# ShuhangGu/DASR

Measured on AMD Instinct MI355X. Metric: SR train images/sec (4x, 128->512), higher is better.
Workload: dtype bf16 MFMA operands, fp32 accumulate / fp32 residual stream

## Files before the change

### dasr_amd/csrc/common.h

```cpp
#pragma once
#include <hip/hip_runtime.h>
#include <hip/hip_ext.h>
#include <stdint.h>
#include "../../include/dasr_hip.h"

typedef __bf16 bf16_t;
typedef __attribute__((ext_vector_type(8))) __bf16 bf16x8;
typedef __attribute__((ext_vector_type(4))) __bf16 bf16x4;
typedef __attribute__((ext_vector_type(4))) short s16x4;
typedef _Float16 f16_t;
typedef __attribute__((ext_vector_type(8))) _Float16 f16x8;
typedef __attribute__((ext_vector_type(4))) _Float16 f16x4;
typedef __attribute__((ext_vector_type(16))) float f32x16;
typedef __attribute__((ext_vector_type(4))) float f32x4;
typedef __attribute__((ext_vector_type(4))) unsigned int u32x4;
typedef __attribute__((ext_vector_type(2))) unsigned int u32x2;

#define DASR_LDS __attribute__((address_space(3)))

#define HIP_TRY(expr)                                   \
    do {                                                \
        hipError_t _e = (expr);                         \
        if (_e != hipSuccess) return (int)_e;           \
    } while (0)

__device__ __forceinline__ float bf16_to_f32(bf16_t v) { return (float)v; }

__device__ __forceinline__ bf16_t f32_to_bf16(float v) { return (bf16_t)v; }

__device__ __forceinline__ void split_bf16(float v, bf16_t& hi, bf16_t& lo) {
    hi = (bf16_t)v;
    lo = (bf16_t)(v - (float)hi);
}

__device__ __forceinline__ void split_f16(float v, bf16_t& hi, bf16_t& lo) {
    const f16_t h = (f16_t)v;
    hi = __builtin_bit_cast(bf16_t, h);
    lo = __builtin_bit_cast(bf16_t, (f16_t)(v - (float)h));
}

template <bool F16>
__device__ __forceinline__ f32x16 mfma16(bf16x8 a, bf16x8 b, f32x16 c) {
    if constexpr (F16) return __builtin_amdgcn_mfma_f32_32x32x16_f16(__builtin_bit_cast(f16x8, a), __builtin_bit_cast(f16x8, b), c, 0, 0, 0);
    else return __builtin_amdgcn_mfma_f32_32x32x16_bf16(a, b, c, 0, 0, 0);
}

__device__ __forceinline__ float wave_sum(float v) {
#pragma unroll
    for (int o = 32; o > 0; o >>= 1) v += __shfl_xor(v, o, 64);
    return v;
}

static inline hipStream_t as_stream(void* s) { return (hipStream_t)s; }

struct dasr_red {
    float* part;
    unsigned* ticket;
};
dasr_red dasr_red_scratch(const void* key_acc, hipStream_t s, unsigned nblocks, int k);
int dasr_red_error();

template <int K>
__device__ __forceinline__ void grid_sum_commit(const dasr_red r, const float (&v)[K], float* const (&acc)[K], const float (&coef)[K]) {
    if (!r.part) return;
    __shared__ unsigned gs_last;
    __shared__ float gs_red[K][4];
    const unsigned nb = gridDim.x;
    if (threadIdx.x == 0) {
#pragma unroll
        for (int k = 0; k < K; ++k) __hip_atomic_store(r.part + (size_t)k * nb + blockIdx.x, v[k], __ATOMIC_RELAXED, __HIP_MEMORY_SCOPE_AGENT);
        asm volatile("s_waitcnt vmcnt(0)" ::: "memory");
        gs_last = __hip_atomic_fetch_add(r.ticket, 1u, __ATOMIC_RELAXED, __HIP_MEMORY_SCOPE_AGENT) == nb - 1u;
    }
    __syncthreads();
    if (!gs_last) return;
#pragma unroll
    for (int k = 0; k < K; ++k) {
        float s = 0.f;
        for (unsigned i = threadIdx.x; i < nb; i += 256u) s += __hip_atomic_load(r.part + (size_t)k * nb + i, __ATOMIC_RELAXED, __HIP_MEMORY_SCOPE_AGENT);
        s = wave_sum(s);
        if ((threadIdx.x & 63) == 0) gs_red[k][threadIdx.x >> 6] = s;
    }
    __syncthreads();
    if (threadIdx.x == 0) {
#pragma unroll
        for (int k = 0; k < K; ++k)
            if (acc[k]) atomicAdd(acc[k], ((gs_red[k][0] + gs_red[k][1]) + (gs_red[k][2] + gs_red[k][3])) * coef[k]);
        __hip_atomic_store(r.ticket, 0u, __ATOMIC_RELAXED, __HIP_MEMORY_SCOPE_AGENT);
    }
}

bool dasr_prof_slot(const char* tag, hipEvent_t* e0, hipEvent_t* e1);
#define DASR_LAUNCH_TAG(tag, kfn, grid, block, lds, s, ...)                                         \
    do {                                                                                            \
        hipEvent_t _e0 = nullptr, _e1 = nullptr;                                                    \
        if (dasr_prof_slot(tag, &_e0, &_e1)) hipExtLaunchKernelGGL(kfn, grid, block, lds, s, _e0, _e1, 0, __VA_ARGS__); \
        else hipLaunchKernelGGL(kfn, grid, block, lds, s, __VA_ARGS__);                             \
    } while (0)
#define DASR_LAUNCH(kfn, ...) DASR_LAUNCH_TAG(#kfn, kfn, __VA_ARGS__)
```

### dasr_amd/csrc/misc.hip

```cpp
#include "common.h"
#include <string.h>
#include <atomic>
#include <condition_variable>
#include <map>
#include <mutex>
#include <thread>
#include <tuple>

namespace {

__global__ void pack_kernel(const dasr_pack_desc* __restrict__ descs, int ndesc, long long total,
                            const long long* __restrict__ prefix, const float* __restrict__ params, bf16_t* __restrict__ packed) {
    const long long gid = (long long)blockIdx.x * blockDim.x + threadIdx.x;
    if (gid >= total) return;
    int lo = 0, hi = ndesc - 1;
    while (lo < hi) {
        const int mid = (lo + hi + 1) >> 1;
        if (prefix[mid] <= gid) lo = mid; else hi = mid - 1;
    }
    const dasr_pack_desc& D = descs[lo];
    long long q = gid - prefix[lo];
    const int lane = q & 63;
    q >>= 6;
    const int mi = q % D.mt;
    q /= D.mt;
    const int tap = q % D.ntaps;
    q /= D.ntaps;
    const int nchunks = D.cin_pad >> 4;
    const int ckv = q % nchunks;
    const int mg = q / nchunks;
    const int oc = (mg * D.mt + mi) * 32 + (lane & 31);
    const int kreal = D.fmt >= 3 ? nchunks / 3 : nchunks;
    const int part = ckv / kreal, ck = ckv - part * kreal;
    const int c0 = ck * 16 + 8 * (lane >> 5);
    bf16x8 vh, vl;
#pragma unroll
    for (int e = 0; e < 8; ++e) {
        const int cin = c0 + e;
        float v = 0.f;
        if (oc < D.cout) {
            for (int s = 0; s < D.nseg; ++s) {
                const dasr_pack_seg& S = D.seg[s];
                const int ci = cin - S.cin_start;
                if (ci >= 0 && ci < S.cin_len) {
                    const int st = D.tapmap[tap];
                    const unsigned msk = tap < 16 ? D.tapmask[tap] : 0u;
                    const bool okc = !S.transpose || ci < S.src_cout;
                    const long long base = !S.transpose ? S.src_off + ((long long)oc * S.src_cin + S.src_c0 + ci) * D.src_ntaps
                                                        : S.src_off + ((long long)ci * S.src_cin + S.src_c0 + oc) * D.src_ntaps;
                    if (msk && okc) {
                        float acc = 0.f;
                        for (int k = 0; k < D.src_ntaps && k < 16; ++k)
                            if (msk & (1u << k)) acc += params[base + k];
                        v = acc;
                    } else if (st >= 0 && okc) {
                        v = params[base + st];
                    }
                }
            }
        }
        bf16_t h, l;
        split_bf16(v, h, l);
        if (D.fmt == 1) h = __builtin_bit_cast(bf16_t, (f16_t)v);
        if (D.fmt == 2 || D.fmt == 3) split_f16(v, h, l);
        if (D.fmt >= 3 && part == 2) h = l;
        vh[e] = h;
        vl[e] = l;
    }
    const long long o = D.dst_off + (gid - prefix[lo]) * 8;
    *(bf16x8*)(packed + o) = vh;
    if (D.lo_off) *(bf16x8*)(packed + o + D.lo_off) = vl;
}

__global__ void nchw_to_blocked_kernel(const float* __restrict__ src, int N, int C, int H, int W, dasr_tensor df, dasr_tensor db) {
    const int ncb = (C + 15) >> 4;
    const long long total = (long long)N * ncb * H * W;
    const long long i = (long long)blockIdx.x * blockDim.x + threadIdx.x;
    if (i >= total) return;
    const int x = i % W;
    long long t = i / W;
    const int y = t % H;
    t /= H;
    const int cb = t % ncb;
    const int n = t / ncb;
    float v[16];
#pragma unroll
    for (int j = 0; j < 16; ++j) {
        const int c = cb * 16 + j;
        v[j] = c < C ? src[(((long long)n * C + c) * H + y) * W + x] : 0.f;
    }
    const size_t po = ((size_t)y * W + x) * 16;
    if (df.p) {
        float* d = (float*)df.p + (size_t)n * df.n_stride + (size_t)cb * df.cb_stride + po;
#pragma unroll
        for (int j = 0; j < 4; ++j) ((f32x4*)d)[j] = f32x4{v[4 * j], v[4 * j + 1], v[4 * j + 2], v[4 * j + 3]};
    }
    if (db.p) {
        bf16_t* d = (bf16_t*)db.p + (size_t)n * db.n_stride + (size_t)cb * db.cb_stride + po;
        bf16x8 a, b;
#pragma unroll
        for (int j = 0; j < 8; ++j) {
            a[j] = (bf16_t)v[j];
            b[j] = (bf16_t)v[8 + j];
        }
        ((bf16x8*)d)[0] = a;
        ((bf16x8*)d)[1] = b;
    }
}

__global__ void blocked_to_nchw_kernel(dasr_tensor s, int N, int C, int H, int W, float* __restrict__ dst) {
    const long long total = (long long)N * C * H * W;
    const long long i = (long long)blockIdx.x * blockDim.x + threadIdx.x;
    if (i >= total) return;
    const int x = i % W;
    long long t = i / W;
    const int y = t % H;
    t /= H;
    const int c = t % C;
    const int n = t / C;
    dst[i] = ((const float*)s.p)[(size_t)n * s.n_stride + (size_t)(c >> 4) * s.cb_stride + ((size_t)y * W + x) * 16 + (c & 15)];
}

__global__ void l1_loss_kernel(dasr_tensor sr, const float* __restrict__ hr, const float* __restrict__ wm, int N, int C, int H, int W,
                               float coef, float* loss_acc, dasr_tensor grad, int accumulate, float gscale, dasr_red rs) {
    const long long total = (long long)N * H * W;
    const long long i = (long long)blockIdx.x * blockDim.x + threadIdx.x;
    float part = 0.f;
    if (i < total) {
        const int x = i % W;
        long long t = i / W;
        const int y = t % H;
        const int n = t / H;
        const size_t po = ((size_t)y * W + x) * 16;
        const float* s = (const float*)sr.p + (size_t)n * sr.n_stride + po;
        const float wgt = wm ? wm[((long long)n * H + y) * W + x] : 1.f;
        float g[16];
#pragma unroll
        for (int j = 0; j < 16; ++j) g[j] = 0.f;
        for (int c = 0; c < C; ++c) {
            const float d = s[c] - hr[(((long long)n * C + c) * H + y) * W + x];
            if (accumulate & 2) {
                part += wgt * d * d;
                g[c] = 2.f * coef * wgt * d;
            } else {
                part += wgt * fabsf(d);
                g[c] = coef * wgt * (d > 0.f ? 1.f : (d < 0.f ? -1.f : 0.f));
            }
        }
        if (grad.p && (accumulate & 4)) {
            f16_t* gp = (f16_t*)grad.p + (size_t)n * grad.n_stride + po;
            for (int j = 0; j < (C + 3) / 4; ++j) {
                f16x4 o;
#pragma unroll
                for (int e = 0; e < 4; ++e) o[e] = (f16_t)(g[4 * j + e] * gscale);
                ((f16x4*)gp)[j] = o;
            }
        } else if (grad.p) {
            float* gp = (float*)grad.p + (size_t)n * grad.n_stride + po;
#pragma unroll
            for (int j = 0; j < 4; ++j) {
                f32x4 o = {g[4 * j], g[4 * j + 1], g[4 * j + 2], g[4 * j + 3]};
                if (accumulate & 1) o += ((const f32x4*)gp)[j];
                ((f32x4*)gp)[j] = o;
            }
        }
    }
    part = wave_sum(part);
    __shared__ float red[4];
    if ((threadIdx.x & 63) == 0) red[threadIdx.x >> 6] = part;
    __syncthreads();
    const float v[1] = {red[0] + red[1] + red[2] + red[3]};
    float* const acc[1] = {loss_acc};
    const float cf[1] = {coef};
    grid_sum_commit<1>(rs, v, acc, cf);
}

__global__ void downsum2x_kernel(dasr_tensor src, int N, int C, int H, int W, dasr_tensor mask, int mask_f32, float slope,
                                 dasr_tensor df, dasr_tensor db) {
    const int ncb = (C + 15) >> 4;
    const long long total = (long long)N * ncb * H * W * 4;
    const long long gi = (long long)blockIdx.x * blockDim.x + threadIdx.x;
    if (gi >= total) return;
    const int q = gi & 3;
    const long long i = gi >> 2;
    const int x = i % W;
    long long t = i / W;
    const int y = t % H;
    t /= H;
    const int cb = t % ncb;
    const int n = t / ncb;
    const float* s = (const float*)src.p + (size_t)n * src.n_stride + (size_t)cb * src.cb_stride + q * 4;
    const int W2 = 2 * W;
    f32x4 a = *(const f32x4*)(s + ((size_t)(2 * y) * W2 + 2 * x) * 16);
    a += *(const f32x4*)(s + ((size_t)(2 * y) * W2 + 2 * x + 1) * 16);
    a += *(const f32x4*)(s + ((size_t)(2 * y + 1) * W2 + 2 * x) * 16);
    a += *(const f32x4*)(s + ((size_t)(2 * y + 1) * W2 + 2 * x + 1) * 16);
    const size_t po = ((size_t)y * W + x) * 16 + q * 4;
    if (mask.p) {
        const size_t mo = (size_t)n * mask.n_stride + (size_t)cb * mask.cb_stride + po;
        float m[4];
        if (mask_f32) {
            const f32x4 mv = *(const f32x4*)((const float*)mask.p + mo);
            for (int j = 0; j < 4; ++j) m[j] = mv[j];
        } else {
            const bf16x4 mv = *(const bf16x4*)((const bf16_t*)mask.p + mo);
            for (int j = 0; j < 4; ++j) m[j] = (float)mv[j];
        }
        for (int j = 0; j < 4; ++j) a[j] = m[j] > 0.f ? a[j] : a[j] * slope;
    }
    if (df.p) *(f32x4*)((float*)df.p + (size_t)n * df.n_stride + (size_t)cb * df.cb_stride + po) = a;
    if (db.p) {
        bf16x4 o;
        for (int j = 0; j < 4; ++j) o[j] = (bf16_t)a[j];
        *(bf16x4*)((bf16_t*)db.p + (size_t)n * db.n_stride + (size_t)cb * db.cb_stride + po) = o;
    }
}

__global__ void axpby_kernel(dasr_tensor x, float a, dasr_tensor z, float b, int N, int C, int H, int W, dasr_tensor of,
                             dasr_tensor ob, float gamma, dasr_tensor mask, float slope, const float* slope_ptr) {
    const int ncb = (C + 15) >> 4;
    const long long per_plane = (long long)H * W * 4;
    const long long total = (long long)N * ncb * per_plane;
    const long long gi = (long long)blockIdx.x * blockDim.x + threadIdx.x;
    if (gi >= total) return;
    const long long e = (gi % per_plane) * 4;
    long long t = gi / per_plane;
    const int cb = t % ncb;
    const int n = t / ncb;
    f32x4 v = *(const f32x4*)((const float*)x.p + (size_t)n * x.n_stride + (size_t)cb * x.cb_stride + e) * a;
    if (z.p) v += *(const f32x4*)((const float*)z.p + (size_t)n * z.n_stride + (size_t)cb * z.cb_stride + e) * b;
    if (mask.p) {
        const float sl = slope_ptr ? *slope_ptr : slope;
        const f32x4 mv = *(const f32x4*)((const float*)mask.p + (size_t)n * mask.n_stride + (size_t)cb * mask.cb_stride + e);
        for (int j = 0; j < 4; ++j) v[j] = mv[j] > 0.f ? v[j] : v[j] * sl;
    }
    if (of.p) *(f32x4*)((float*)of.p + (size_t)n * of.n_stride + (size_t)cb * of.cb_stride + e) = v;
    if (ob.p) {
        bf16x4 o;
        for (int j = 0; j < 4; ++j) o[j] = (bf16_t)(v[j] * gamma);
        *(bf16x4*)((bf16_t*)ob.p + (size_t)n * ob.n_stride + (size_t)cb * ob.cb_stride + e) = o;
    }
}

__global__ void adam_kernel(float* __restrict__ p, const float* __restrict__ g, float* __restrict__ m, float* __restrict__ v,
                            long long n, float step_size, float beta1, float beta2, float eps, float wd, float inv_sqrt_bc2, int* __restrict__ nonfinite,
                            const int* __restrict__ gate) {
    if (gate && *gate != 0) return;
    bool bad = false;
    for (long long i = (long long)blockIdx.x * blockDim.x + threadIdx.x; i < n; i += (long long)gridDim.x * blockDim.x) {
        float gi = g[i];
        bad |= !(fabsf(gi) <= 3.0e38f);
        const float pi = p[i];
        if (wd != 0.f) gi += wd * pi;
        const float mi = beta1 * m[i] + (1.f - beta1) * gi;
        const float vi = beta2 * v[i] + (1.f - beta2) * gi * gi;
        m[i] = mi;
        v[i] = vi;
        const float denom = sqrtf(vi) * inv_sqrt_bc2 + eps;
        p[i] = pi - step_size * (mi / denom);
    }
    if (nonfinite && __any(bad) && (threadIdx.x & 63) == 0) atomicOr(nonfinite, 1);
}

__global__ void add_flat_kernel(float* __restrict__ y, const float* __restrict__ x, long long n) {
    for (long long i = (long long)blockIdx.x * blockDim.x + threadIdx.x; i < n; i += (long long)gridDim.x * blockDim.x) y[i] += x[i];
}

__global__ void fill_kernel(float* p, long long n, float v) {
    for (long long i = (long long)blockIdx.x * blockDim.x + threadIdx.x; i < n; i += (long long)gridDim.x * blockDim.x) p[i] = v;
}

inline unsigned blocks_for(long long total, int bs = 256) { return (unsigned)((total + bs - 1) / bs); }

}

extern "C" int dasr_pack_weights(const dasr_pack_desc* descs_dev, int32_t ndesc, int64_t total_pieces, const int64_t* piece_prefix_dev,
                                 const float* params_flat, void* packed, void* stream) {
    if (ndesc <= 0 || total_pieces <= 0) return DASR_EINVAL;
    DASR_LAUNCH(pack_kernel, dim3(blocks_for(total_pieces)), dim3(256), 0, as_stream(stream), descs_dev, ndesc,
                       (long long)total_pieces, (const long long*)piece_prefix_dev, params_flat, (bf16_t*)packed);
    return (int)hipGetLastError();
}

extern "C" int dasr_nchw_to_blocked(const float* src, int32_t N, int32_t C, int32_t H, int32_t W, dasr_tensor dst_f32,
                                    dasr_tensor dst_bf16, void* stream) {
    const long long total = (long long)N * ((C + 15) / 16) * H * W;
    if (total <= 0) return DASR_EINVAL;
    DASR_LAUNCH(nchw_to_blocked_kernel, dim3(blocks_for(total)), dim3(256), 0, as_stream(stream), src, N, C, H, W, dst_f32, dst_bf16);
    return (int)hipGetLastError();
}

extern "C" int dasr_blocked_to_nchw(dasr_tensor src, int32_t N, int32_t C, int32_t H, int32_t W, float* dst, void* stream) {
    const long long total = (long long)N * C * H * W;
    if (total <= 0) return DASR_EINVAL;
    DASR_LAUNCH(blocked_to_nchw_kernel, dim3(blocks_for(total)), dim3(256), 0, as_stream(stream), src, N, C, H, W, dst);
    return (int)hipGetLastError();
}

extern "C" int dasr_l1_loss(dasr_tensor sr, const float* hr_nchw, const float* weight_map, int32_t N, int32_t C, int32_t H, int32_t W,
                            float coef, float* loss_acc, dasr_tensor grad, int32_t accumulate, float grad_scale, void* stream) {
    const long long total = (long long)N * H * W;
    if (total <= 0 || C > 16) return DASR_EINVAL;
    if ((accumulate & 4) && (accumulate & 1)) return DASR_EINVAL;
    const dasr_red rs = dasr_red_scratch(loss_acc, as_stream(stream), blocks_for(total), 1);
    if (loss_acc && !rs.part) return dasr_red_error();
    DASR_LAUNCH(l1_loss_kernel, dim3(blocks_for(total)), dim3(256), 0, as_stream(stream), sr, hr_nchw, weight_map, N, C, H, W, coef,
                       loss_acc, grad, accumulate, grad_scale != 0.f ? grad_scale : 1.f, rs);
    return (int)hipGetLastError();
}

extern "C" int dasr_downsum2x(dasr_tensor src, int32_t N, int32_t C, int32_t H, int32_t W, dasr_tensor mask, int32_t mask_f32,
                              float slope, dasr_tensor dst_f32, dasr_tensor dst_bf16, void* stream) {
    const long long total = (long long)N * ((C + 15) / 16) * H * W * 4;
    if (total <= 0) return DASR_EINVAL;
    DASR_LAUNCH(downsum2x_kernel, dim3(blocks_for(total)), dim3(256), 0, as_stream(stream), src, N, C, H, W, mask, mask_f32, slope,
                       dst_f32, dst_bf16);
    return (int)hipGetLastError();
}

__device__ __forceinline__ float f32_rounded(float v) {
    asm("" : "+v"(v));
    return v;
}

__global__ void cvt_f16_kernel(dasr_tensor x, int N, int C, int H, int W, float scale, dasr_tensor y) {
    const int ncb = (C + 15) >> 4;
    const long long per_plane = (long long)H * W * 4, total = (long long)N * ncb * per_plane;
    const long long gi = (long long)blockIdx.x * blockDim.x + threadIdx.x;
    if (gi >= total) return;
    const long long e = (gi % per_plane) * 4;
    long long t = gi / per_plane;
    const int cb = t % ncb, n = t / ncb;
    const f32x4 v = *(const f32x4*)((const float*)x.p + (size_t)n * x.n_stride + (size_t)cb * x.cb_stride + e);
    f16x4 o;
    for (int j = 0; j < 4; ++j) o[j] = (f16_t)f32_rounded(v[j] * scale);
    *(f16x4*)((f16_t*)y.p + (size_t)n * y.n_stride + (size_t)cb * y.cb_stride + e) = o;
}

__global__ void f16_residual_kernel(dasr_tensor x, int N, int C, int H, int W, float scale, dasr_tensor y) {
    const int ncb = (C + 15) >> 4;
    const long long per_plane = (long long)H * W * 4, total = (long long)N * ncb * per_plane;
    const long long gi = (long long)blockIdx.x * blockDim.x + threadIdx.x;
    if (gi >= total) return;
    const long long e = (gi % per_plane) * 4;
    long long t = gi / per_plane;
    const int cb = t % ncb, n = t / ncb;
    const f32x4 v = *(const f32x4*)((const float*)x.p + (size_t)n * x.n_stride + (size_t)cb * x.cb_stride + e);
    const float inv = 1.f / scale;
    f32x4 o;
    for (int j = 0; j < 4; ++j) o[j] = v[j] - (float)(f16_t)f32_rounded(v[j] * scale) * inv;
    *(f32x4*)((float*)y.p + (size_t)n * y.n_stride + (size_t)cb * y.cb_stride + e) = o;
}

template <typename T>
__global__ void cvt_split16_kernel(dasr_tensor x, int N, int C, int H, int W, float scale, dasr_tensor y) {
    const int ncb = (C + 15) >> 4;
    const long long per_plane = (long long)H * W * 4, total = (long long)N * ncb * per_plane;
    const long long gi = (long long)blockIdx.x * blockDim.x + threadIdx.x;
    if (gi >= total) return;
    const long long e = (gi % per_plane) * 4;
    long long t = gi / per_plane;
    const int cb = t % ncb, n = t / ncb;
    const f32x4 v = *(const f32x4*)((const float*)x.p + (size_t)n * x.n_stride + (size_t)cb * x.cb_stride + e);
    T* yp = (T*)y.p + (size_t)n * y.n_stride + (size_t)cb * y.cb_stride + e;
    const size_t lo = (size_t)ncb * y.cb_stride;
#pragma unroll
    for (int j = 0; j < 4; ++j) {
        const float vv = f32_rounded(v[j] * scale);
        const T h = (T)vv;
        yp[j] = h;
        yp[lo + j] = (T)(vv - (float)h);
    }
}

__global__ void downsum2x_f16_kernel(dasr_tensor src, int N, int C, int H, int W, dasr_tensor mask, float slope, float out_scale, dasr_tensor df,
                                     dasr_tensor dh) {
    const int ncb = (C + 15) >> 4;
    const long long total = (long long)N * ncb * H * W * 4;
    const long long gi = (long long)blockIdx.x * blockDim.x + threadIdx.x;
    if (gi >= total) return;
    const int q = gi & 3;
    const long long i = gi >> 2;
    const int x = i % W;
    long long t = i / W;
    const int y = t % H;
    t /= H;
    const int cb = t % ncb, n = t / ncb;
    const f16_t* s = (const f16_t*)src.p + (size_t)n * src.n_stride + (size_t)cb * src.cb_stride + q * 4;
    const int W2 = 2 * W;
    float a[4] = {0.f, 0.f, 0.f, 0.f};
    for (int dy = 0; dy < 2; ++dy)
        for (int dx = 0; dx < 2; ++dx) {
            const f16x4 v = *(const f16x4*)(s + ((size_t)(2 * y + dy) * W2 + 2 * x + dx) * 16);
            for (int j = 0; j < 4; ++j) a[j] += (float)v[j];
        }
    const size_t po = ((size_t)y * W + x) * 16 + q * 4;
    if (mask.p) {
        const f16x4 mv = *(const f16x4*)((const f16_t*)mask.p + (size_t)n * mask.n_stride + (size_t)cb * mask.cb_stride + po);
        for (int j = 0; j < 4; ++j) a[j] = (float)mv[j] > 0.f ? a[j] : a[j] * slope;
    }
    for (int j = 0; j < 4; ++j) a[j] *= out_scale;
    if (df.p) *(f32x4*)((float*)df.p + (size_t)n * df.n_stride + (size_t)cb * df.cb_stride + po) = f32x4{a[0], a[1], a[2], a[3]};
    if (dh.p) {
        f16x4 o;
        for (int j = 0; j < 4; ++j) o[j] = (f16_t)a[j];
        *(f16x4*)((f16_t*)dh.p + (size_t)n * dh.n_stride + (size_t)cb * dh.cb_stride + po) = o;
    }
}

__global__ void pixel_shuffle_f16_kernel(dasr_tensor src, int N, int C4, int H, int W, dasr_tensor dst) {
    const int ncb = C4 >> 4;
    const long long total = (long long)N * ncb * H * W;
    const long long i = (long long)blockIdx.x * blockDim.x + threadIdx.x;
    if (i >= total) return;
    const int x = i % W;
    long long t = i / W;
    const int y = t % H;
    t /= H;
    const int p = t % ncb, n = t / ncb;
    const f16_t* s = (const f16_t*)src.p + (size_t)n * src.n_stride + (size_t)p * src.cb_stride + ((size_t)y * W + x) * 16;
    const f16x8 lo = *(const f16x8*)s, hi = *(const f16x8*)(s + 8);
    f16_t v[16];
    for (int j = 0; j < 8; ++j) { v[j] = lo[j]; v[8 + j] = hi[j]; }
    f16_t* d = (f16_t*)dst.p + (size_t)n * dst.n_stride + (size_t)(p >> 2) * dst.cb_stride + 4 * (p & 3);
    const int W2 = 2 * W;
    for (int k = 0; k < 4; ++k) {
        const f16x4 o = {v[k], v[4 + k], v[8 + k], v[12 + k]};
        *(f16x4*)(d + ((size_t)(2 * y + (k >> 1)) * W2 + 2 * x + (k & 1)) * 16) = o;
    }
}

__global__ void pixel_unshuffle_f16_kernel(dasr_tensor gsrc, dasr_tensor mask, float slope, int N, int C4, int H, int W, dasr_tensor gdst) {
    const int ncb = C4 >> 4;
    const long long total = (long long)N * ncb * H * W;
    const long long i = (long long)blockIdx.x * blockDim.x + threadIdx.x;
    if (i >= total) return;
    const int x = i % W;
    long long t = i / W;
    const int y = t % H;
    t /= H;
    const int p = t % ncb, n = t / ncb;
    const f16_t* g = (const f16_t*)gsrc.p + (size_t)n * gsrc.n_stride + (size_t)(p >> 2) * gsrc.cb_stride + 4 * (p & 3);
    const int W2 = 2 * W;
    f16_t v[16];
    for (int k = 0; k < 4; ++k) {
        const f16x4 q = *(const f16x4*)(g + ((size_t)(2 * y + (k >> 1)) * W2 + 2 * x + (k & 1)) * 16);
        for (int cc = 0; cc < 4; ++cc) v[4 * cc + k] = q[cc];
    }
    const size_t po = (size_t)n * gdst.n_stride + (size_t)p * gdst.cb_stride + ((size_t)y * W + x) * 16;
    if (mask.p) {
        const f16_t* m = (const f16_t*)mask.p + (size_t)n * mask.n_stride + (size_t)p * mask.cb_stride + ((size_t)y * W + x) * 16;
        for (int j = 0; j < 16; ++j) v[j] = (float)m[j] > 0.f ? v[j] : (f16_t)((float)v[j] * slope);
    }
    f16x8 lo, hi;
    for (int j = 0; j < 8; ++j) { lo[j] = v[j]; hi[j] = v[8 + j]; }
    *(f16x8*)((f16_t*)gdst.p + po) = lo;
    *(f16x8*)((f16_t*)gdst.p + po + 8) = hi;
}

extern "C" int dasr_pixel_shuffle_f16(dasr_tensor src, int32_t N, int32_t C4, int32_t H, int32_t W, dasr_tensor dst, void* stream) {
    const long long total = (long long)N * (C4 / 16) * H * W;
    if (total <= 0 || (C4 & 63) || !src.p || !dst.p) return DASR_EINVAL;
    DASR_LAUNCH(pixel_shuffle_f16_kernel, dim3(blocks_for(total)), dim3(256), 0, as_stream(stream), src, N, C4, H, W, dst);
    return (int)hipGetLastError();
}

extern "C" int dasr_pixel_unshuffle_f16(dasr_tensor gsrc, dasr_tensor mask, float slope, int32_t N, int32_t C4, int32_t H, int32_t W, dasr_tensor gdst,
                                        void* stream) {
    const long long total = (long long)N * (C4 / 16) * H * W;
    if (total <= 0 || (C4 & 63) || !gsrc.p || !gdst.p) return DASR_EINVAL;
    DASR_LAUNCH(pixel_unshuffle_f16_kernel, dim3(blocks_for(total)), dim3(256), 0, as_stream(stream), gsrc, mask, slope, N, C4, H, W, gdst);
    return (int)hipGetLastError();
}

extern "C" int dasr_cvt_f16(dasr_tensor x, int32_t N, int32_t C, int32_t H, int32_t W, float scale, dasr_tensor y, void* stream) {
    const long long total = (long long)N * ((C + 15) / 16) * H * W * 4;
    if (total <= 0 || !x.p || !y.p) return DASR_EINVAL;
    DASR_LAUNCH(cvt_f16_kernel, dim3(blocks_for(total)), dim3(256), 0, as_stream(stream), x, N, C, H, W, scale, y);
    return (int)hipGetLastError();
}

extern "C" int dasr_cvt_split16(dasr_tensor x, int32_t N, int32_t C, int32_t H, int32_t W, float scale, dasr_tensor y, int32_t f16, void* stream) {
    const long long total = (long long)N * ((C + 15) / 16) * H * W * 4;
    if (total <= 0 || !x.p || !y.p) return DASR_EINVAL;
    if (f16) DASR_LAUNCH(cvt_split16_kernel<f16_t>, dim3(blocks_for(total)), dim3(256), 0, as_stream(stream), x, N, C, H, W, scale, y);
    else DASR_LAUNCH(cvt_split16_kernel<bf16_t>, dim3(blocks_for(total)), dim3(256), 0, as_stream(stream), x, N, C, H, W, scale, y);
    return (int)hipGetLastError();
}

extern "C" int dasr_f16_residual(dasr_tensor x, int32_t N, int32_t C, int32_t H, int32_t W, float scale, dasr_tensor y, void* stream) {
    const long long total = (long long)N * ((C + 15) / 16) * H * W * 4;
    if (total <= 0 || !x.p || !y.p || !(scale > 0.f)) return DASR_EINVAL;
    DASR_LAUNCH(f16_residual_kernel, dim3(blocks_for(total)), dim3(256), 0, as_stream(stream), x, N, C, H, W, scale, y);
    return (int)hipGetLastError();
}

extern "C" int dasr_downsum2x_f16(dasr_tensor src, int32_t N, int32_t C, int32_t H, int32_t W, dasr_tensor mask, float slope, float out_scale,
                                  dasr_tensor dst_f32, dasr_tensor dst_f16, void* stream) {
    const long long total = (long long)N * ((C + 15) / 16) * H * W * 4;
    if (total <= 0 || !src.p) return DASR_EINVAL;
    DASR_LAUNCH(downsum2x_f16_kernel, dim3(blocks_for(total)), dim3(256), 0, as_stream(stream), src, N, C, H, W, mask, slope, out_scale, dst_f32, dst_f16);
    return (int)hipGetLastError();
}

extern "C" int dasr_axpby(dasr_tensor x, float a, dasr_tensor z, float b, int32_t N, int32_t C, int32_t H, int32_t W,
                          dasr_tensor out_f32, dasr_tensor out_bf16, float gamma, dasr_tensor mask, float slope, const float* slope_ptr,
                          void* stream) {
    const long long total = (long long)N * ((C + 15) / 16) * H * W * 4;
    if (total <= 0) return DASR_EINVAL;
    DASR_LAUNCH(axpby_kernel, dim3(blocks_for(total)), dim3(256), 0, as_stream(stream), x, a, z, b, N, C, H, W, out_f32, out_bf16, gamma, mask, slope, slope_ptr);
    return (int)hipGetLastError();
}

extern "C" int dasr_adam(float* p, const float* g, float* m, float* v, int64_t n, float lr, float beta1, float beta2, float eps,
                         float weight_decay, int32_t step, int32_t* nonfinite_flag, const int32_t* gate_flag, void* stream) {
    if (n <= 0 || step <= 0) return DASR_EINVAL;
    const double bc1 = 1.0 - pow((double)beta1, (double)step), bc2 = 1.0 - pow((double)beta2, (double)step);
    const float step_size = (float)((double)lr / bc1);
    const float inv_sqrt_bc2 = (float)(1.0 / sqrt(bc2));
    const unsigned blocks = (unsigned)((n + 255) / 256 < 4096 ? (n + 255) / 256 : 4096);
    DASR_LAUNCH(adam_kernel, dim3(blocks), dim3(256), 0, as_stream(stream), p, g, m, v, (long long)n, step_size, beta1, beta2, eps,
                       weight_decay, inv_sqrt_bc2, nonfinite_flag, gate_flag);
    return (int)hipGetLastError();
}

extern "C" int dasr_fill_f32(float* p, int64_t n, float value, void* stream) {
    if (n <= 0) return DASR_EINVAL;
    const unsigned blocks = (unsigned)((n + 255) / 256 < 4096 ? (n + 255) / 256 : 4096);
    DASR_LAUNCH(fill_kernel, dim3(blocks), dim3(256), 0, as_stream(stream), p, (long long)n, value);
    return (int)hipGetLastError();
}

extern "C" int dasr_add_flat(float* y, const float* x, int64_t n, void* stream) {
    if (n <= 0) return DASR_EINVAL;
    const unsigned blocks = (unsigned)((n + 255) / 256 < 4096 ? (n + 255) / 256 : 4096);
    DASR_LAUNCH(add_flat_kernel, dim3(blocks), dim3(256), 0, as_stream(stream), y, x, (long long)n);
    return (int)hipGetLastError();
}

__global__ void gather_crops_kernel(const dasr_crop_desc* __restrict__ descs, int n, int C, int size, float* __restrict__ dst) {
    const long long total = (long long)n * C * size * size;
    const long long i = (long long)blockIdx.x * blockDim.x + threadIdx.x;
    if (i >= total) return;
    const int x = i % size;
    long long t = i / size;
    const int y = t % size;
    t /= size;
    const int c = t % C;
    const int k = t / C;
    const dasr_crop_desc D = descs[k];
    int ci = y, cj = x;
    if (D.flags & 4) { ci = x; cj = y; }
    if (D.flags & 2) ci = size - 1 - ci;
    if (D.flags & 1) cj = size - 1 - cj;
    const int vy = D.y0 + ci, vx = D.x0 + cj;
    float v = 0.f;
    if (c < D.C && vy >= 0 && vy < D.vH && vx >= 0 && vx < D.vW) {
        const float* s = D.src + (size_t)c * D.H * D.W;
        if (D.vH == D.H && D.vW == D.W) {
            v = s[(size_t)vy * D.W + vx];
        } else {
            float fy = ((float)vy + 0.5f) * ((float)D.H / (float)D.vH) - 0.5f, fx = ((float)vx + 0.5f) * ((float)D.W / (float)D.vW) - 0.5f;
            int y0 = (int)floorf(fy), x0 = (int)floorf(fx);
            const float wy = fy - (float)y0, wx = fx - (float)x0;
            const int y1 = min(max(y0 + 1, 0), D.H - 1), x1 = min(max(x0 + 1, 0), D.W - 1);
            y0 = min(max(y0, 0), D.H - 1);
            x0 = min(max(x0, 0), D.W - 1);
            v = (1.f - wy) * ((1.f - wx) * s[(size_t)y0 * D.W + x0] + wx * s[(size_t)y0 * D.W + x1]) +
                wy * ((1.f - wx) * s[(size_t)y1 * D.W + x0] + wx * s[(size_t)y1 * D.W + x1]);
        }
    }
    dst[i] = v;
}

extern "C" int dasr_gather_crops(const dasr_crop_desc* descs_dev, int32_t n, int32_t C, int32_t size, float* dst, void* stream) {
    const long long total = (long long)n * C * size * size;
    if (n <= 0 || C <= 0 || size <= 0 || !descs_dev || !dst) return DASR_EINVAL;
    DASR_LAUNCH(gather_crops_kernel, dim3((unsigned)((total + 255) / 256)), dim3(256), 0, as_stream(stream), descs_dev, n, C, size, dst);
    return (int)hipGetLastError();
}

extern "C" void* dasr_event_create(void) {
    hipEvent_t e = nullptr;
    if (hipEventCreateWithFlags(&e, hipEventDisableTiming) != hipSuccess) return nullptr;
    return (void*)e;
}

extern "C" int dasr_event_destroy(void* ev) { return ev ? (int)hipEventDestroy((hipEvent_t)ev) : 0; }

extern "C" int dasr_abi_version(void) { return DASR_ABI_VERSION; }

static thread_local int g_last_failed_op = -1;
extern "C" int dasr_last_failed_op(void) { return g_last_failed_op; }

namespace {
struct RedRow {
    char* base;
    size_t floats;
};
std::mutex g_red_mu;
std::map<std::tuple<int, const void*, hipStream_t>, RedRow> g_red_rows;
thread_local bool g_red_capture_refused = false;
}

int dasr_red_error() {
    const bool c = g_red_capture_refused;
    g_red_capture_refused = false;
    return c ? DASR_ECAPTURE : DASR_EINVAL;
}

// ... 334 lines not shown
```

Baseline: 535.8.

## Restructure weight pack and L1 loss kernels for per-row reuse and fewer blocks

The weight pack kernel now uses a wave-wide ballot search to find the descriptor. For small-tap filters, one wave loads each source row once and writes every tap from registers, instead of one thread per tap re-reading params. The L1 loss kernel processes 16 virtual blocks per real block with unrolled loads, and C<=4 gets its own specialisation. A new row-based grid reduction keeps the same per-virtual-block partial layout. Both changes cut launch count and redundant loads, but they add code complexity and per-thread register pressure.

```diff
diff --git a/dasr_amd/csrc/common.h b/dasr_amd/csrc/common.h
--- a/dasr_amd/csrc/common.h
+++ b/dasr_amd/csrc/common.h
@@ -90,6 +90,38 @@
     }
 }
 
+template <int K>
+__device__ __forceinline__ void grid_sum_commit_rows(const dasr_red r, const float (&v)[K], unsigned vb0, unsigned nv, unsigned nvb, float* const (&acc)[K],
+                                                     const float (&coef)[K]) {
+    if (!r.part) return;
+    __shared__ unsigned gsr_last;
+    __shared__ float gsr_red[K][4];
+    if (threadIdx.x < 64) {
+        if (threadIdx.x < nv) {
+#pragma unroll
+            for (int k = 0; k < K; ++k) __hip_atomic_store(r.part + (size_t)k * nvb + vb0 + threadIdx.x, v[k], __ATOMIC_RELAXED, __HIP_MEMORY_SCOPE_AGENT);
+        }
+        asm volatile("s_waitcnt vmcnt(0)" ::: "memory");
+        if (threadIdx.x == 0) gsr_last = __hip_atomic_fetch_add(r.ticket, 1u, __ATOMIC_RELAXED, __HIP_MEMORY_SCOPE_AGENT) == gridDim.x - 1u;
+    }
+    __syncthreads();
+    if (!gsr_last) return;
+#pragma unroll
+    for (int k = 0; k < K; ++k) {
+        float s = 0.f;
+        for (unsigned i = threadIdx.x; i < nvb; i += 256u) s += __hip_atomic_load(r.part + (size_t)k * nvb + i, __ATOMIC_RELAXED, __HIP_MEMORY_SCOPE_AGENT);
+        s = wave_sum(s);
+        if ((threadIdx.x & 63) == 0) gsr_red[k][threadIdx.x >> 6] = s;
+    }
+    __syncthreads();
+    if (threadIdx.x == 0) {
+#pragma unroll
+        for (int k = 0; k < K; ++k)
+            if (acc[k]) atomicAdd(acc[k], ((gsr_red[k][0] + gsr_red[k][1]) + (gsr_red[k][2] + gsr_red[k][3])) * coef[k]);
+        __hip_atomic_store(r.ticket, 0u, __ATOMIC_RELAXED, __HIP_MEMORY_SCOPE_AGENT);
+    }
+}
+
 bool dasr_prof_slot(const char* tag, hipEvent_t* e0, hipEvent_t* e1);
 #define DASR_LAUNCH_TAG(tag, kfn, grid, block, lds, s, ...)                                         \
     do {                                                                                            \
diff --git a/dasr_amd/csrc/misc.hip b/dasr_amd/csrc/misc.hip
--- a/dasr_amd/csrc/misc.hip
+++ b/dasr_amd/csrc/misc.hip
@@ -9,67 +9,157 @@
 
 namespace {
 
-__global__ void pack_kernel(const dasr_pack_desc* __restrict__ descs, int ndesc, long long total,
-                            const long long* __restrict__ prefix, const float* __restrict__ params, bf16_t* __restrict__ packed) {
-    const long long gid = (long long)blockIdx.x * blockDim.x + threadIdx.x;
-    if (gid >= total) return;
-    int lo = 0, hi = ndesc - 1;
-    while (lo < hi) {
-        const int mid = (lo + hi + 1) >> 1;
-        if (prefix[mid] <= gid) lo = mid; else hi = mid - 1;
+
+__device__ __forceinline__ long long pack_src_base(const dasr_pack_seg (&S)[5], int nseg, int cout, int src_ntaps, int oc, int cin) {
+    long long base = -1;
+    if (oc < cout) {
+#pragma unroll
+        for (int s = 0; s < 5; ++s) {
+            const int ci = cin - S[s].cin_start;
+            if (s < nseg && ci >= 0 && ci < S[s].cin_len) {
+                const bool okc = !S[s].transpose || ci < S[s].src_cout;
+                if (okc)
+                    base = !S[s].transpose ? S[s].src_off + ((long long)oc * S[s].src_cin + S[s].src_c0 + ci) * src_ntaps
+                                           : S[s].src_off + ((long long)ci * S[s].src_cin + S[s].src_c0 + oc) * src_ntaps;
+            }
+        }
+    }
+    return base;
+}
+
+__device__ __forceinline__ void pack_round(int fmt, int part, float v, bf16_t& h, bf16_t& l) {
+    split_bf16(v, h, l);
+    if (fmt == 1) h = __builtin_bit_cast(bf16_t, (f16_t)v);
+    if (fmt == 2 || fmt == 3) split_f16(v, h, l);
+    if (fmt >= 3 && part == 2) h = l;
+}
+
+template <int SN, int E>
+__device__ __forceinline__ void pack_rows(const dasr_pack_desc& D, const dasr_pack_seg (&S)[5], const float* __restrict__ params,
+                                          bf16_t* __restrict__ packed, long long o0, int oc, int c0, int part) {
+    typedef __attribute__((ext_vector_type(E))) __bf16 piece_t;
+    const int lane = threadIdx.x & 63;
+    const int st_l = D.tapmap[lane & 31];
+    const int mk_l = D.tapmask[lane & 15];
+    const long long tap_stride = (long long)D.mt * 64 * 8;
+#pragma unroll 1
+    for (int e0 = 0; e0 < 8; e0 += E) {
+        float w[E][SN];
+#pragma unroll
+        for (int e = 0; e < E; ++e) {
+            const long long base = pack_src_base(S, D.nseg, D.cout, D.src_ntaps, oc, c0 + e0 + e);
+#pragma unroll
+            for (int k = 0; k < SN; ++k) w[e][k] = 0.f;
+            if (base >= 0 && D.src_ntaps == SN) {
+                typedef float row4_t __attribute__((ext_vector_type(4), aligned(4)));
+                const row4_t* rp = (const row4_t*)(params + base);
+#pragma unroll
+                for (int k4 = 0; k4 < SN / 4; ++k4) {
+                    const row4_t r = rp[k4];
+#pragma unroll
+                    for (int j = 0; j < 4; ++j) w[e][4 * k4 + j] = r[j];
+                }
+#pragma unroll
+                for (int k = SN / 4 * 4; k < SN; ++k) w[e][k] = params[base + k];
+            } else if (base >= 0) {
+#pragma unroll
+                for (int k = 0; k < SN; ++k)
+                    if (k < D.src_ntaps) w[e][k] = params[base + k];
+            }
+        }
+        for (int t = 0; t < D.ntaps; ++t) {
+            const int st = __builtin_amdgcn_readlane(st_l, t);
+            const unsigned msk = t < 16 ? (unsigned)__builtin_amdgcn_readlane(mk_l, t) : 0u;
+            piece_t vh, vl;
+#pragma unroll
+            for (int e = 0; e < E; ++e) {
+                float v = 0.f;
+                if (msk) {
+                    float acc = 0.f;
+#pragma unroll
+                    for (int k = 0; k < SN; ++k)
+                        if (k < D.src_ntaps && (msk & (1u << k))) acc += w[e][k];
+                    v = acc;
+                } else if (st >= 0) {
+#pragma unroll
+                    for (int k = 0; k < SN; ++k) v = k == st ? w[e][k] : v;
+                }
+                bf16_t h, l;
+                pack_round(D.fmt, part, v, h, l);
+                vh[e] = h;
+                vl[e] = l;
+            }
+            const long long o = o0 + t * tap_stride + e0;
+            *(piece_t*)(packed + o) = vh;
+            if (D.lo_off) *(piece_t*)(packed + o + D.lo_off) = vl;
+        }
+    }
+}
+
+__global__ __launch_bounds__(256) void pack_kernel(const dasr_pack_desc* __restrict__ descs, int ndesc, long long total,
+                                                   const long long* __restrict__ prefix, const float* __restrict__ params, bf16_t* __restrict__ packed) {
+    const long long g0 = (long long)blockIdx.x * 256 + (__builtin_amdgcn_readfirstlane((int)threadIdx.x) & ~63);
+    if (g0 >= total) return;
+    int lo = 0, n = ndesc;
+    while (n > 1) {
+        const int stride = (n + 63) >> 6;
+        const int idx = lo + (int)(threadIdx.x & 63) * stride;
+        const bool le = idx < lo + n && prefix[idx] <= g0;
+        const int c = __builtin_popcountll(__ballot(le));
+        const int end = lo + n;
+        lo += (c - 1) * stride;
+        n = end - lo < stride ? end - lo : stride;
     }
     const dasr_pack_desc& D = descs[lo];
-    long long q = gid - prefix[lo];
-    const int lane = q & 63;
-    q >>= 6;
-    const int mi = q % D.mt;
-    q /= D.mt;
-    const int tap = q % D.ntaps;
-    q /= D.ntaps;
+    const long long p0 = g0 - prefix[lo];
+    unsigned q = (unsigned)(p0 >> 6);
+    const int mi = q % (unsigned)D.mt;
+    q /= (unsigned)D.mt;
+    const int tap = q % (unsigned)D.ntaps;
+    q /= (unsigned)D.ntaps;
     const int nchunks = D.cin_pad >> 4;
-    const int ckv = q % nchunks;
-    const int mg = q / nchunks;
+    const int ckv = q % (unsigned)nchunks;
+    const int mg = q / (unsigned)nchunks;
+    const bool rows = D.src_ntaps <= 16;
+    if (rows && tap != 0) return;
+    const int lane = threadIdx.x & 63;
     const int oc = (mg * D.mt + mi) * 32 + (lane & 31);
     const int kreal = D.fmt >= 3 ? nchunks / 3 : nchunks;
     const int part = ckv / kreal, ck = ckv - part * kreal;
     const int c0 = ck * 16 + 8 * (lane >> 5);
+    const long long o0 = D.dst_off + (p0 + lane) * 8;
+    dasr_pack_seg S[5];
+#pragma unroll
+    for (int s = 0; s < 5; ++s) S[s] = D.seg[s];
+    if (rows) {
+        if (D.src_ntaps <= 9) pack_rows<9, 8>(D, S, params, packed, o0, oc, c0, part);
+        else pack_rows<16, 4>(D, S, params, packed, o0, oc, c0, part);
+        return;
+    }
+    const int st = D.tapmap[tap];
     bf16x8 vh, vl;
 #pragma unroll
     for (int e = 0; e < 8; ++e) {
-        const int cin = c0 + e;
+        const long long base = pack_src_base(S, D.nseg, D.cout, D.src_ntaps, oc, c0 + e);
         float v = 0.f;
-        if (oc < D.cout) {
-            for (int s = 0; s < D.nseg; ++s) {
-                const dasr_pack_seg& S = D.seg[s];
-                const int ci = cin - S.cin_start;
-                if (ci >= 0 && ci < S.cin_len) {
-                    const int st = D.tapmap[tap];
-                    const unsigned msk = tap < 16 ? D.tapmask[tap] : 0u;
-                    const bool okc = !S.transpose || ci < S.src_cout;
-                    const long long base = !S.transpose ? S.src_off + ((long long)oc * S.src_cin + S.src_c0 + ci) * D.src_ntaps
-                                                        : S.src_off + ((long long)ci * S.src_cin + S.src_c0 + oc) * D.src_ntaps;
-                    if (msk && okc) {
-                        float acc = 0.f;
-                        for (int k = 0; k < D.src_ntaps && k < 16; ++k)
-                            if (msk & (1u << k)) acc += params[base + k];
-                        v = acc;
-                    } else if (st >= 0 && okc) {
-                        v = params[base + st];
-                    }
-                }
+        if (base >= 0) {
+            const unsigned msk = tap < 16 ? D.tapmask[tap] : 0u;
+            if (msk) {
+                float acc = 0.f;
+                for (int k = 0; k < 16; ++k)
+                    if (msk & (1u << k)) acc += params[base + k];
+                v = acc;
+            } else if (st >= 0) {
+                v = params[base + st];
             }
         }
         bf16_t h, l;
-        split_bf16(v, h, l);
-        if (D.fmt == 1) h = __builtin_bit_cast(bf16_t, (f16_t)v);
-        if (D.fmt == 2 || D.fmt == 3) split_f16(v, h, l);
-        if (D.fmt >= 3 && part == 2) h = l;
+        pack_round(D.fmt, part, v, h, l);
         vh[e] = h;
         vl[e] = l;
     }
-    const long long o = D.dst_off + (gid - prefix[lo]) * 8;
-    *(bf16x8*)(packed + o) = vh;
-    if (D.lo_off) *(bf16x8*)(packed + o + D.lo_off) = vl;
+    *(bf16x8*)(packed + o0) = vh;
+    if (D.lo_off) *(bf16x8*)(packed + o0 + D.lo_off) = vl;
 }
 
 __global__ void nchw_to_blocked_kernel(const float* __restrict__ src, int N, int C, int H, int W, dasr_tensor df, dasr_tensor db) {
@@ -121,58 +211,109 @@
     dst[i] = ((const float*)s.p)[(size_t)n * s.n_stride + (size_t)(c >> 4) * s.cb_stride + ((size_t)y * W + x) * 16 + (c & 15)];
 }
 
-__global__ void l1_loss_kernel(dasr_tensor sr, const float* __restrict__ hr, const float* __restrict__ wm, int N, int C, int H, int W,
-                               float coef, float* loss_acc, dasr_tensor grad, int accumulate, float gscale, dasr_red rs) {
-    const long long total = (long long)N * H * W;
-    const long long i = (long long)blockIdx.x * blockDim.x + threadIdx.x;
-    float part = 0.f;
-    if (i < total) {
-        const int x = i % W;
-        long long t = i / W;
-        const int y = t % H;
-        const int n = t / H;
-        const size_t po = ((size_t)y * W + x) * 16;
-        const float* s = (const float*)sr.p + (size_t)n * sr.n_stride + po;
-        const float wgt = wm ? wm[((long long)n * H + y) * W + x] : 1.f;
-        float g[16];
-#pragma unroll
-        for (int j = 0; j < 16; ++j) g[j] = 0.f;
-        for (int c = 0; c < C; ++c) {
-            const float d = s[c] - hr[(((long long)n * C + c) * H + y) * W + x];
-            if (accumulate & 2) {
-                part += wgt * d * d;
-                g[c] = 2.f * coef * wgt * d;
-            } else {
-                part += wgt * fabsf(d);
-                g[c] = coef * wgt * (d > 0.f ? 1.f : (d < 0.f ? -1.f : 0.f));
-            }
-        }
-        if (grad.p && (accumulate & 4)) {
-            f16_t* gp = (f16_t*)grad.p + (size_t)n * grad.n_stride + po;
-            for (int j = 0; j < (C + 3) / 4; ++j) {
+constexpr int L1_V = 16;
+constexpr int L1_U = 4;
+static_assert(L1_U == 4 && L1_V % L1_U == 0 && L1_V <= 64, "grid_sum_commit_rows stores the partials from wave 0");
+
+__device__ __forceinline__ void l1_term(float d, float wgt, float coef, bool squared, float& part, float& g) {
+    if (squared) {
+        part += wgt * d * d;
+        g = 2.f * coef * wgt * d;
+    } else {
+        part += wgt * fabsf(d);
+        g = coef * wgt * (d > 0.f ? 1.f : (d < 0.f ? -1.f : 0.f));
+    }
+}
+
+__device__ __forceinline__ void l1_pixel_of(int nb, unsigned r, unsigned HW, int W, int& n, int& y, int& x) {
+    const unsigned dn = r / HW;
+    n = nb + (int)dn;
+    r -= dn * HW;
+    y = (int)(r / (unsigned)W);
+    x = (int)(r - (unsigned)y * (unsigned)W);
+}
+
+template <int G>
+__device__ __forceinline__ void l1_store_grad(const float (&g)[4 * G], const dasr_tensor& grad, int n, size_t po, int C, int accumulate, float gscale) {
+    if (grad.p && (accumulate & 4)) {
+        f16_t* gp = (f16_t*)grad.p + (size_t)n * grad.n_stride + po;
+#pragma unroll
+        for (int j = 0; j < G; ++j) {
+            if (j < (C + 3) / 4) {
                 f16x4 o;
 #pragma unroll
                 for (int e = 0; e < 4; ++e) o[e] = (f16_t)(g[4 * j + e] * gscale);
                 ((f16x4*)gp)[j] = o;
             }
-        } else if (grad.p) {
-            float* gp = (float*)grad.p + (size_t)n * grad.n_stride + po;
-#pragma unroll
-            for (int j = 0; j < 4; ++j) {
-                f32x4 o = {g[4 * j], g[4 * j + 1], g[4 * j + 2], g[4 * j + 3]};
-                if (accumulate & 1) o += ((const f32x4*)gp)[j];
-                ((f32x4*)gp)[j] = o;
+        }
+    } else if (grad.p) {
+        float* gp = (float*)grad.p + (size_t)n * grad.n_stride + po;
+#pragma unroll
+        for (int j = 0; j < 4; ++j) {
+            f32x4 o = {0.f, 0.f, 0.f, 0.f};
+            if (j < G) o = f32x4{g[4 * j], g[4 * j + 1], g[4 * j + 2], g[4 * j + 3]};
+            if (accumulate & 1) o += ((const f32x4*)gp)[j];
+            ((f32x4*)gp)[j] = o;
+        }
+    }
+}
+
+template <int G>
+__global__ __launch_bounds__(256) void l1_loss_kernel(dasr_tensor sr, const float* __restrict__ hr, const float* __restrict__ wm, int N, int C, int H, int W,
+                                                      float coef, float* loss_acc, dasr_tensor grad, int accumulate, float gscale, dasr_red rs, unsigned nvb) {
+    constexpr int U = L1_U / G;
+    const long long total = (long long)N * H * W;
+    const unsigned vb0 = blockIdx.x * (unsigned)L1_V;
+    const unsigned nv = nvb - vb0 < (unsigned)L1_V ? nvb - vb0 : (unsigned)L1_V;
+    const bool squared = accumulate & 2;
+    const unsigned HW = (unsigned)H * (unsigned)W;
+    __shared__ float red[L1_V][4];
+    for (unsigned v = 0; v < nv; v += U) {
+        const long long ib = (long long)(vb0 + v) * 256;
+        const int nb = ib / HW;
+        const unsigned rb = (unsigned)(ib - (long long)nb * HW);
+        const unsigned last = (unsigned)(total - 1 - ib < (long long)(U * 256) ? total - 1 - ib : (long long)(U * 256));
+        bool in[U];
+        int n[U];
+        size_t po[U];
+        f32x4 s[U][G];
+        float h[U][4 * G], wgt[U];
+#pragma unroll
+        for (int u = 0; u < U; ++u) {
+            const unsigned t = threadIdx.x + u * 256;
+            in[u] = t <= last;
+            int y, x;
+            l1_pixel_of(nb, rb + (in[u] ? t : last), HW, W, n[u], y, x);
+            po[u] = ((size_t)y * W + x) * 16;
+            const f32x4* sp = (const f32x4*)((const float*)sr.p + (size_t)n[u] * sr.n_stride + po[u]);
+#pragma unroll
+            for (int j = 0; j < G; ++j) s[u][j] = sp[j];
+#pragma unroll
+            for (int c = 0; c < 4 * G; ++c) h[u][c] = hr[(((long long)n[u] * C + (c < C ? c : C - 1)) * H + y) * W + x];
+            wgt[u] = *(wm ? wm + (((long long)n[u] * H + y) * W + x) : hr);
+        }
+#pragma unroll
+        for (int u = 0; u < U; ++u) {
+            float part = 0.f;
+            if (in[u]) {
+                const float w1 = wm ? wgt[u] : 1.f;
+                float g[4 * G];
+#pragma unroll
+                for (int c = 0; c < 4 * G; ++c) {
+                    g[c] = 0.f;
+                    if (c < C) l1_term(s[u][c >> 2][c & 3] - h[u][c], w1, coef, squared, part, g[c]);
+                }
+                l1_store_grad<G>(g, grad, n[u], po[u], C, accumulate, gscale);
             }
-        }
-    }
-    part = wave_sum(part);
-    __shared__ float red[4];
-    if ((threadIdx.x & 63) == 0) red[threadIdx.x >> 6] = part;
+            part = wave_sum(part);
+            if ((threadIdx.x & 63) == 0) red[v + u][threadIdx.x >> 6] = part;
+        }
+    }
     __syncthreads();
-    const float v[1] = {red[0] + red[1] + red[2] + red[3]};
+    const float pv[1] = {threadIdx.x < nv ? red[threadIdx.x][0] + red[threadIdx.x][1] + red[threadIdx.x][2] + red[threadIdx.x][3] : 0.f};
     float* const acc[1] = {loss_acc};
     const float cf[1] = {coef};
-    grid_sum_commit<1>(rs, v, acc, cf);
+    grid_sum_commit_rows<1>(rs, pv, vb0, nv, nvb, acc, cf);
 }
 
 __global__ void downsum2x_kernel(dasr_tensor src, int N, int C, int H, int W, dasr_tensor mask, int mask_f32, float slope,
@@ -302,10 +443,17 @@
     const long long total = (long long)N * H * W;
     if (total <= 0 || C > 16) return DASR_EINVAL;
     if ((accumulate & 4) && (accumulate & 1)) return DASR_EINVAL;
-    const dasr_red rs = dasr_red_scratch(loss_acc, as_stream(stream), blocks_for(total), 1);
+    const unsigned nvb = blocks_for(total);
+    const dasr_red rs = dasr_red_scratch(loss_acc, as_stream(stream), nvb, 1);
     if (loss_acc && !rs.part) return dasr_red_error();
-    DASR_LAUNCH(l1_loss_kernel, dim3(blocks_for(total)), dim3(256), 0, as_stream(stream), sr, hr_nchw, weight_map, N, C, H, W, coef,
-                       loss_acc, grad, accumulate, grad_scale != 0.f ? grad_scale : 1.f, rs);
+    const dim3 grid((nvb + L1_V - 1) / L1_V);
+    const float gs = grad_scale != 0.f ? grad_scale : 1.f;
+    if (C <= 4)
+        DASR_LAUNCH_TAG("l1_loss_kernel", l1_loss_kernel<1>, grid, dim3(256), 0, as_stream(stream), sr, hr_nchw, weight_map, N, C, H, W, coef, loss_acc, grad,
+                        accumulate, gs, rs, nvb);
+    else
+        DASR_LAUNCH_TAG("l1_loss_kernel", l1_loss_kernel<4>, grid, dim3(256), 0, as_stream(stream), sr, hr_nchw, weight_map, N, C, H, W, coef, loss_acc, grad,
+                        accumulate, gs, rs, nvb);
     return (int)hipGetLastError();
 }
 
```

Result: no change. 539.5 (median of 6 runs) (+0.7%).
